# GothiProCoder/OCR-System

Measured on AMD Instinct MI355X. Metric: pages/sec end-to-end det+rec, A4@200DPI, higher is better.
Workload: dtype bf16; 1 GPU; end-to-end det+rec, batch=64 A4@200DPI pages per GPU (BASELINE configs[3]); pages_per_gpu=64, global_batch=64, lines_last_step=3279, pages_gathered_last_step=64, parallelism=pages sharded dp1, 1 all-gather/step, ranks=1, input=pages pre-decoded (uint8 RGB) and resident in HBM when the timed region starts, det_sub_batch=64

## Files before the change

### ocr-system_amd/csrc/capi.hip

```cpp
#include <cstdlib>
#include <cstring>
#include <new>

#include "../../include/lumina_ocr.h"
#include "dbpost.h"
#include "deskew.h"
#include "engine.h"
#include "marks.h"
#include "barcodes.h"
#include "qrcodes.h"
#include "datamatrix.h"
#include "aztec.h"
#include "ops.h"
#include "orient.h"
#include "resize.h"
#include "runs.h"
#include "jpeg.h"
#include "jpegdec.h"
#include "lzw.h"
#include "pngdec.h"
#include "ccitt.h"
#include "stem_conv.h"
#include "tables.h"

// ... 67 lines not shown
    return for_page_groups(h, n, fit_group(h->post_group, n, ws), ws, [&](int b0, int nb) {
        CodeGroup<T> g{};
        g.rgb = pages_dev + (size_t)b0 * height * width * 3; g.nb = nb;
        g.codes = codes_dev + (size_t)b0 * max_codes * 12; g.data = data_dev + (size_t)b0 * max_codes * row_len; g.counts = counts_dev + b0;
        g.slot_counts = slot_counts_dev ? slot_counts_dev + b0 : nullptr;
        g.mask_in = mask_in_dev ? reinterpret_cast<const unsigned long long*>(mask_in_dev) + (size_t)b0 * height * nw : nullptr;
        g.mask_out = mask_out_dev ? reinterpret_cast<unsigned long long*>(mask_out_dev) + (size_t)b0 * height * nw : nullptr;
        return hip_rc(h, what, launch(g, h->ws.get(), h->ws.cap));
    });
    API_CATCH(h)
}

extern "C" {

const char* lumina_ocr_version(void) { return "lumina-ocr-mi355x 0.1 (gfx950)"; }

int lumina_ocr_create(int device, lumina_ocr_t** out) {
    if (!out) return 1;
    *out = nullptr;
    lumina_ocr* eng = new (std::nothrow) lumina_ocr();
    if (!eng) return 1;
    eng->device = device;
    int ndev = 0;
    if (hipGetDeviceCount(&ndev) != hipSuccess || device < 0 || device >= ndev) {
        eng->err = "no HIP device " + std::to_string(device) + " (device count " + std::to_string(ndev) + ")";
        *out = eng;
        return 2;
    }
    if (hipSetDevice(device) != hipSuccess) { eng->err = "hipSetDevice failed"; *out = eng; return 2; }
    if (const char* e = getenv("LUMINA_RING_ORIENT")) eng->ring_orient = atoi(e) < 0 ? -1 : (atoi(e) != 0);
    if (getenv("LUMINA_CONV_NO_RING")) eng->conv_ring = false;
    if (getenv("LUMINA_BLOCKED")) eng->blocked_layout = atoi(getenv("LUMINA_BLOCKED")) != 0;
    *out = eng;
    return 0;
}

void lumina_ocr_destroy(lumina_ocr_t* h) {
    if (!h) return;
    (void)hipSetDevice(h->device);
    delete h;
}

const char* lumina_ocr_last_error(const lumina_ocr_t* h) { return h ? h->err.c_str() : "null handle"; }

int lumina_ocr_set_option(lumina_ocr_t* h, const char* key, int value) {
    if (!h || !key) return 1;
    if (!strcmp(key, "det_sub_batch")) h->det_sub_batch = value > 0 ? value : 1;
    else if (!strcmp(key, "rec_sub_batch")) h->rec_sub_batch = value > 0 ? value : 1;
    else if (!strcmp(key, "cls_sub_batch")) h->cls_sub_batch = value > 0 ? value : 1;
    else if (!strcmp(key, "keep_taps")) h->keep_taps = value < 0 || value > 2 ? 0 : value;
    else if (!strcmp(key, "time_convs")) h->time_convs = value != 0;
    else if (!strcmp(key, "fuse_head")) h->fuse_head = value != 0;
    else if (!strcmp(key, "fuse_mb")) h->fuse_mb = value != 0;
    else if (!strcmp(key, "fuse_pool")) h->fuse_pool = value != 0;
    else if (!strcmp(key, "fuse_stem")) h->fuse_stem = value != 0;
    else if (!strcmp(key, "fpn_multi")) h->fpn_multi = value != 0;
    else if (!strcmp(key, "fpn_compose")) h->fpn_compose = value != 0;
    else if (!strcmp(key, "fuse_short")) h->fuse_short = value != 0;
    else if (!strcmp(key, "conv_ring")) h->conv_ring = value != 0;
    else if (!strcmp(key, "blocked_layout")) h->blocked_layout = value != 0;
    else if (!strcmp(key, "conv_big_min")) h->conv_big_min = value >= 0 ? value : 1024;
    else if (!strcmp(key, "ring_orient")) h->ring_orient = value < 0 ? -1 : (value != 0);
    else if (!strcmp(key, "post_group")) h->post_group = value > 0 ? value : 1;
    else if (!strcmp(key, "tail_group")) h->tail_group = value > 0 ? value : 0;
    else if (!strcmp(key, "svtr_f16")) h->svtr_f16 = value < 0 ? -1 : (value != 0);
    else if (!strcmp(key, "png_sub_batch_mb")) h->pd_sub_batch_mb = value > 0 ? value : 1;
    else if (!strcmp(key, "conv2d_variant")) h->conv2d_variant = value < 0 || value > 2 ? 0 : value;
    else return locr_fail(h, "set_option: unknown key", key);
    return 0;
}

int lumina_ocr_load_det_weights(lumina_ocr_t* h, const void* blob, size_t nbytes) {
    if (!h || !blob) return 1;
    BIND(h);
    API_TRY return eng_load_det(h, blob, nbytes); API_CATCH(h)
}
int lumina_ocr_load_rec_weights(lumina_ocr_t* h, const void* blob, size_t nbytes) {
    if (!h || !blob) return 1;
    BIND(h);
    API_TRY return eng_load_rec(h, blob, nbytes); API_CATCH(h)
}
int lumina_ocr_num_classes(const lumina_ocr_t* h) { return h ? h->num_classes : 0; }

int lumina_ocr_normalize(lumina_ocr_t* h, const uint8_t* img_dev, int n, int height, int width, int hp, int wp, const float scale[3],
                         const float shift[3], int layout_nchw, uint16_t* out_dev, void* stream) {
    if (!h || !img_dev || !out_dev || hp < height || wp < width) return locr_fail(h, "normalize", "bad arguments");
    BIND(h);
    return hip_rc(h, "normalize", normalize_launch(img_dev, out_dev, n, height, width, hp, wp, height, width, scale, shift, layout_nchw, (hipStream_t)stream));
}

int lumina_ocr_det_forward(lumina_ocr_t* h, const uint8_t* pages_dev, int batch, int height, int width, int hp, int wp, uint16_t* prob_dev,
                           void* stream) {
    if (!h || !pages_dev || !prob_dev) return locr_fail(h, "det_forward", "null argument");
    BIND(h);
    API_TRY return eng_det_forward(h, pages_dev, batch, height, width, hp, wp, prob_dev, (hipStream_t)stream); API_CATCH(h)
}

int lumina_ocr_det_postprocess(lumina_ocr_t* h, const uint16_t* prob_dev, int batch, int hp, int wp, int valid_h, int valid_w, float thresh,
                               float box_thresh, float unclip_ratio, int min_size, int max_boxes, int32_t* boxes_dev, float* scores_dev,
                               int32_t* counts_dev, void* stream) {
    if (!h || !prob_dev || !boxes_dev || !scores_dev || !counts_dev) return locr_fail(h, "det_postprocess", "null argument");
    if (batch <= 0 || max_boxes <= 0 || valid_h > hp || valid_w > wp) return locr_fail(h, "det_postprocess", "bad dimensions");
    BIND(h);
    API_TRY
    return for_page_groups(h, batch, h->post_group, [&](int nb) { return dbpost_workspace_bytes(nb, hp, wp, max_boxes); }, [&](int b0, int nb) {
        DbPostParams p{};
// ... 750 lines not shown
```

### ocr-system_amd/csrc/conv_mfma.h

```cpp
#pragma once
#include "common.h"

enum ConvOutMode : int {
    OUT_NORMAL = 0,
    OUT_UPSAMPLE = 1,
    OUT_CONVT = 2,
    OUT_CONVT1 = 3,
    OUT_POOL = 4,
};

struct ConvParams {
    const bf16_t* x;
    const bf16_t* wpk;
    const float* bias;
    const bf16_t* res;
    bf16_t* y;
    int N, H, W, Cin;
    int Ho, Wo;
    int Cout;
    int y_cstride, y_coff;
    int res_cstride, res_h, res_w, res_shift;
    int act;
    int out_mode, up_shift, convt_c;
    int tiles_x, tiles_y, n_tiles;
    const bf16_t* fuse_w;
    float fuse_b;
    const bf16_t* gate;
    int gate_hw;
    int dbg_skip;
    int pix_limit;
    const bf16_t* zeros;
    int x_blk, y_blk, res_blk;
    int n_src;
    const bf16_t* xs[4];
    int xs_shift[4];
    int xs_nchunk[4], xs_cstride[4];
    const bf16_t* wpk2;
    const float* bias2;
    bf16_t* y2;
    int y2_cstride;
};

struct ConvKernelCfg {
    int ks, stride, bn, ck, tw, nw;
};

size_t conv_packed_weight_elems(int cout_gemm, int ks, int cin, int bn);
void pack_conv_weights(const bf16_t* ohwi, int cout_gemm, int ks, int cin, int bn, int ck, bf16_t* out, int row_major = 0);

bool conv_pick_cfg(int ks, int stride, int cin, int cout_gemm, ConvKernelCfg* cfg);
hipError_t conv_launch(const ConvKernelCfg& cfg, ConvParams p, hipStream_t stream);
const char* conv_kernel_name(const ConvKernelCfg& cfg);

bool conv_ring_supported(const ConvKernelCfg& cfg, const ConvParams& p);
bool conv_ring_transposed(const ConvParams& p, int orientation);
hipError_t conv_ring_launch(ConvParams p, int orientation, hipStream_t stream);
const char* conv_ring_kernel_name(const ConvParams& p, int orientation);

bool conv_pw_supported(const ConvKernelCfg& cfg, const ConvParams& p);
hipError_t conv_pw_launch(const ConvParams& p, hipStream_t stream);
```

### ocr-system_amd/csrc/conv_mfma.hip

```cpp
#include "conv_mfma.h"

#include <cstdlib>

namespace {

template <int KS, int S, int BN, int CK, int TW, int NW = 4, int DB = 0, int MT = 2>
struct Cfg {
    static constexpr int NTHR = NW * 64;
    static constexpr bool DMA = (DB == 3 || DB == 4);
    static constexpr bool POOL = (DB == 4);
    static constexpr bool SC = (DB == 5);
    static_assert(!SC || (KS == 3 && S == 2 && CK == 16), "fused shortcut: the 3x3 / stride-2 block-entry kernel");
    static constexpr int TH = NW * MT;
    static constexpr int PAD = (KS == 3) ? 1 : 0;
    static constexpr int HH = (TH - 1) * S + KS;
    static constexpr int HW = (TW - 1) * S + KS;
    static constexpr int HWP = HW;
    static constexpr int NPL = CK / 8;
    static constexpr int HPX = HH * HWP;
    static constexpr int PMOD = (NPL >= 8) ? 2 : 4;
    static constexpr int PLANE_A = HPX + ((PMOD - HPX % 16) + 16) % 16;
    static constexpr int TAPS = KS * KS;
    static constexpr int WROWS = TAPS * BN;
    static constexpr int PLANE_W = WROWS;
    static constexpr int NT = BN / 32;
    static constexpr int A_BYTES = DMA ? HPX * NPL * 16 : PLANE_A * NPL * 16;
    static constexpr int W_BYTES = PLANE_W * NPL * 16;
    static constexpr int W2_ROWS = SC ? 4 * BN : 0, W2_ITEMS = W2_ROWS * NPL, W2IT = (W2_ITEMS + NTHR - 1) / NTHR, W2_BYTES = W2_ITEMS * 16;
    static constexpr int A_PIX = DMA ? NPL * 16 : 16, A_SL = DMA ? 16 : PLANE_A * 16;
    static constexpr int W_ROW = DMA ? NPL * 16 : 16, W_SL = DMA ? 16 : PLANE_W * 16;
    static constexpr int STAGE_PITCH = BN * 2 + 16;
    static constexpr int STAGE_BYTES = TH * TW * STAGE_PITCH;
    static constexpr int BUF_BYTES = A_BYTES + W_BYTES + W2_BYTES;
    static constexpr int LDS_BYTES = (BUF_BYTES * (DMA ? 2 : 1)) > STAGE_BYTES ? (BUF_BYTES * (DMA ? 2 : 1)) : STAGE_BYTES;
    static_assert(!DMA || (CK == 16 && KS == 3 && S == 1), "DMA variant: 3x3 / stride 1 / 16-channel chunks");
    static constexpr int A_ITEMS = HH * HW * NPL;
    static constexpr int AIT = (A_ITEMS + NTHR - 1) / NTHR;
    static constexpr int W_ITEMS = WROWS * NPL;
    static constexpr int WIT = (W_ITEMS + NTHR - 1) / NTHR;
    static constexpr int CPP = BN / 8;
};

__device__ __forceinline__ bf16x8_t lds_frag(const unsigned char* p) { return *reinterpret_cast<const bf16x8_t*>(p); }

__device__ __forceinline__ uint32_t mul_bf16x2(uint32_t a, uint32_t b) {
    const float lo = __uint_as_float(a << 16) * __uint_as_float(b << 16);
    const float hi = __uint_as_float(a & 0xFFFF0000u) * __uint_as_float(b & 0xFFFF0000u);
    return pack_bf16x2(lo, hi);
}
__device__ __forceinline__ uint4 mul_bf16x8(uint4 a, uint4 b) {
    return make_uint4(mul_bf16x2(a.x, b.x), mul_bf16x2(a.y, b.y), mul_bf16x2(a.z, b.z), mul_bf16x2(a.w, b.w));
}

template <int KS, int S, int BN, int CK, int TW, int NW, int DB, int MT>
__global__ __launch_bounds__(NW * 64, (BN <= 64 ? 2 : 1)) void conv_mfma_kernel(const ConvParams p) {
    using C = Cfg<KS, S, BN, CK, TW, NW, DB, MT>;
    constexpr int NTHR = C::NTHR;
    extern __shared__ __attribute__((aligned(16))) unsigned char smem[];

    const int tid = threadIdx.x, lane = tid & 63, wave = tid >> 6;
    unsigned char* sA = smem;
    unsigned char* sW = sA + C::A_BYTES;
    const int r = lane & 31, h = lane >> 5;

    const int lid = xcd_remap(blockIdx.x, gridDim.x);
    const int ntile = lid % p.n_tiles;
    const int mtile = lid / p.n_tiles;
    const int tiles_per_img = p.tiles_x * p.tiles_y;
    const int n_img = mtile / tiles_per_img;
    const int trem = mtile - n_img * tiles_per_img;
    const int tile_y = trem / p.tiles_x, tile_x = trem - tile_y * p.tiles_x;

    const bf16_t* ximg = p.x + (size_t)n_img * p.H * p.W * p.Cin;
    const int nchunks = p.Cin / CK;
    const bf16_t* wbase = p.wpk + (size_t)ntile * nchunks * C::W_ITEMS * 8;

    const bool blk_dbg = CK == 16 && (p.dbg_skip & 8);
    const int pstride = blk_dbg ? 16 : p.Cin;
    const int cadv = blk_dbg ? p.H * p.W * 16 : CK;
    int a_goff[C::AIT], a_loff[C::AIT];
    int a_gate[KS == 1 ? C::AIT : 1];
    constexpr bool pool = C::POOL;
    const int oyb = pool ? tile_y * (C::TH - 2) - 1 : tile_y * C::TH, oxb = pool ? tile_x * (TW - 2) - 1 : tile_x * TW;
    const int iy0 = oyb * S - C::PAD, ix0 = oxb * S - C::PAD;
#pragma unroll
    for (int it = 0; it < C::AIT; ++it) {
        const int i = tid + NTHR * it;
        const int pi = i / C::NPL, c = i - pi * C::NPL;
        const int hy = pi / C::HW, hx = pi - hy * C::HW;
        const int iy = iy0 + hy, ix = ix0 + hx;
        const bool item = i < C::A_ITEMS;
        const bool inb = item && iy >= 0 && iy < p.H && ix >= 0 && ix < p.W && (p.pix_limit == 0 || iy * p.W + ix < p.pix_limit);
        a_goff[it] = inb ? (iy * p.W + ix) * pstride + c * 8 : -1;
        a_loff[it] = item ? (c * C::PLANE_A + hy * C::HWP + hx) * 16 : -1;
        if constexpr (KS == 1) a_gate[it] = (inb && p.gate != nullptr) ? ((iy * p.W + ix) / p.gate_hw) * p.Cin + c * 8 : -1;
    }

    uint4 a_reg[C::AIT], w_reg[C::WIT];
    uint4 g_reg[KS == 1 ? C::AIT : 1];
    uint4 w2_reg[C::SC ? C::W2IT : 1];
    unsigned char* sW2 = sW + C::W_BYTES;
    const bf16_t* wbase2 = C::SC ? p.wpk2 + (size_t)ntile * nchunks * C::W2_ITEMS * 8 : nullptr;
#define ISSUE_LOADS(chunk_)                                                                          \
    {                                                                                                \
        const bf16_t* xa = ximg + (chunk_) * cadv;                                                   \
        const bool skipa_ = (p.dbg_skip & 2) && (chunk_) > 0, skipw_ = (p.dbg_skip & 1) && (chunk_) > 0; \
        _Pragma("unroll") for (int it = 0; it < C::AIT; ++it) {                                      \
            uint4 t_ = make_uint4(0, 0, 0, 0);                                                       \
            if (a_goff[it] >= 0 && !skipa_) t_ = *reinterpret_cast<const uint4*>(xa + a_goff[it]);   \
            a_reg[it] = t_;                                                                          \
            if constexpr (KS == 1) {                                                                 \
                uint4 g_ = make_uint4(0, 0, 0, 0);                                                   \
                if (a_gate[it] >= 0) g_ = *reinterpret_cast<const uint4*>(p.gate + a_gate[it] + (chunk_) * CK); \
                g_reg[it] = g_;                                                                      \
            }                                                                                        \
        }                                                                                            \
        const uint4* wsrc = reinterpret_cast<const uint4*>(wbase + (size_t)(chunk_) * C::W_ITEMS * 8); \
        _Pragma("unroll") for (int it = 0; it < C::WIT; ++it) {                                      \
            const int i = tid + NTHR * it;                                                          \
            uint4 t_ = make_uint4(0, 0, 0, 0);                                                       \
            if ((C::W_ITEMS % NTHR == 0 || i < C::W_ITEMS) && !skipw_) t_ = wsrc[i];                 \
            w_reg[it] = t_;                                                                          \
        }                                                                                            \
        if constexpr (C::SC) {                                                                       \
// ... 293 lines not shown
                        const int cy = oyb + lr, cx = oxb + lc;
                        if (cy < 0 || cy >= p.Ho || cx < 0 || cx >= p.Wo) continue;
                        const uint4 v = *reinterpret_cast<const uint4*>(stage + (lr * TW + lc) * C::STAGE_PITCH + ch * 16);
                        const uint32_t w4[4] = {v.x, v.y, v.z, v.w};
#pragma unroll
                        for (int j = 0; j < 4; ++j) {
                            m[2 * j] = fmaxf(m[2 * j], __uint_as_float(w4[j] << 16));
                            m[2 * j + 1] = fmaxf(m[2 * j + 1], __uint_as_float(w4[j] & 0xFFFF0000u));
                        }
                    }
                const uint4 o = make_uint4(pack_bf16x2(m[0], m[1]), pack_bf16x2(m[2], m[3]), pack_bf16x2(m[4], m[5]), pack_bf16x2(m[6], m[7]));
                *reinterpret_cast<uint4*>(p.y + (((size_t)n_img * Hq + py) * Wq + px) * p.y_cstride + p.y_coff + co) = o;
            }
            return;
        }
    }
#pragma unroll
    for (int k = 0; k < (C::TH * TW * C::CPP + NTHR - 1) / NTHR; ++k) {
        const int i = tid + NTHR * k;
        const int tp = i / C::CPP, ch = i - tp * C::CPP;
        if (tp >= C::TH * TW) continue;
        const int ty = tp / TW, tx = tp - ty * TW;
        const int oy = oyb + ty, ox = oxb + tx;
        const int co = ntile * BN + ch * 8;
        if (oy >= p.Ho || ox >= p.Wo || co >= cout_r8 || (p.pix_limit != 0 && oy * p.Wo + ox >= p.pix_limit)) continue;
        const uint4 v = *reinterpret_cast<const uint4*>(stage + tp * C::STAGE_PITCH + ch * 16);
        if (p.out_mode == OUT_NORMAL) {
            bf16_t* dst = p.y + (((size_t)n_img * p.Ho + oy) * p.Wo + ox) * p.y_cstride + p.y_coff + co;
            *reinterpret_cast<uint4*>(dst) = v;
        } else if (p.out_mode == OUT_UPSAMPLE) {
            const int f = 1 << p.up_shift;
            const int HoU = p.Ho << p.up_shift, WoU = p.Wo << p.up_shift;
            for (int dy = 0; dy < f; ++dy)
                for (int dx = 0; dx < f; ++dx) {
                    bf16_t* dst = p.y + (((size_t)n_img * HoU + (oy * f + dy)) * WoU + (ox * f + dx)) * p.y_cstride + p.y_coff + co;
                    *reinterpret_cast<uint4*>(dst) = v;
                }
        } else if (p.out_mode == OUT_CONVT) {
            const int q = co / p.convt_c, cc = co - q * p.convt_c;
            const int yy = 2 * oy + (q >> 1), xx = 2 * ox + (q & 1);
            bf16_t* dst = p.y + (((size_t)n_img * (2 * p.Ho) + yy) * (2 * p.Wo) + xx) * p.y_cstride + p.y_coff + cc;
            *reinterpret_cast<uint4*>(dst) = v;
        } else {
            if (ch == 0) {
                bf16_t* dst = p.y + ((size_t)n_img * (2 * p.Ho) + 2 * oy) * (size_t)(2 * p.Wo) + 2 * ox;
                *reinterpret_cast<uint32_t*>(dst) = v.x;
                *reinterpret_cast<uint32_t*>(dst + 2 * p.Wo) = v.y;
            }
        }
    }
}

template <int KS, int S, int BN, int CK, int TW, int NW = 4, int DB = 0, int MT = 2>
hipError_t launch_t(const ConvParams& p, hipStream_t stream) {
    using C = Cfg<KS, S, BN, CK, TW, NW, DB, MT>;
    auto kern = conv_mfma_kernel<KS, S, BN, CK, TW, NW, DB, MT>;
    { hipError_t e = locr_dyn_lds(reinterpret_cast<const void*>(kern), C::LDS_BYTES); if (e != hipSuccess) return e; }
    const int grid = p.N * p.tiles_x * p.tiles_y * p.n_tiles;
    hipLaunchKernelGGL(kern, dim3(grid), dim3(C::NTHR), C::LDS_BYTES, stream, p);
    return hipGetLastError();
}

}

size_t conv_packed_weight_elems(int cout_gemm, int ks, int cin, int bn) {
    const int ntiles = (cout_gemm + bn - 1) / bn;
    return (size_t)ntiles * bn * ks * ks * cin;
}

void pack_conv_weights(const bf16_t* ohwi, int cout_gemm, int ks, int cin, int bn, int ck, bf16_t* out, int row_major) {
    const int ntiles = (cout_gemm + bn - 1) / bn, taps = ks * ks, npl = ck / 8, nchunks = cin / ck;
    const size_t wrows = (size_t)taps * bn;
    if (row_major) {
        for (int nt = 0; nt < ntiles; ++nt)
            for (int chunk = 0; chunk < nchunks; ++chunk)
                for (int tap = 0; tap < taps; ++tap)
                    for (int n = 0; n < bn; ++n) {
                        const int co = nt * bn + n;
                        bf16_t* dst = out + (((size_t)nt * nchunks + chunk) * wrows + (size_t)tap * bn + n) * ck;
                        for (int j = 0; j < ck; ++j)
                            dst[j] = co < cout_gemm ? ohwi[((size_t)co * taps + tap) * cin + chunk * ck + j] : (bf16_t)0;
                    }
        return;
    }
    for (int nt = 0; nt < ntiles; ++nt)
        for (int chunk = 0; chunk < nchunks; ++chunk)
            for (int c = 0; c < npl; ++c)
                for (int tap = 0; tap < taps; ++tap)
                    for (int n = 0; n < bn; ++n) {
                        const int co = nt * bn + n;
                        bf16_t* dst = out + ((((size_t)nt * nchunks + chunk) * npl + c) * wrows + (size_t)tap * bn + n) * 8;
                        for (int j = 0; j < 8; ++j)
                            dst[j] = co < cout_gemm ? ohwi[((size_t)co * taps + tap) * cin + chunk * ck + c * 8 + j] : (bf16_t)0;
                    }
}

bool conv_pick_cfg(int ks, int stride, int cin, int cout_gemm, ConvKernelCfg* cfg) {
    if (!((ks == 1 && stride == 1) || (ks == 2 && stride == 2) || (ks == 3 && (stride == 1 || stride == 2)))) return false;
    if (cin % 16 != 0) return false;
    cfg->ks = ks; cfg->stride = stride; cfg->tw = 32; cfg->nw = 4;
    cfg->ck = (cin % 32 == 0) ? 32 : 16;
    cfg->bn = cout_gemm <= 32 ? 32 : (cout_gemm <= 64 ? 64 : 128);
    if (cfg->bn == 128) cfg->bn = 64;
    if (ks == 3 && stride == 2 && cfg->bn == 128 && cfg->ck == 32) cfg->bn = 64;
    if (stride == 2) cfg->ck = 16;
    if (const char* e = getenv("LUMINA_CONV_CKS2")) { if (stride == 2) cfg->ck = atoi(e) == 32 && cin % 32 == 0 ? 32 : 16; }
    if (ks == 3 && stride == 1 && cin == 32 && cfg->bn == 32) cfg->ck = 16;
    if (const char* e = getenv("LUMINA_CONV_CK3")) { if (ks == 3 && stride == 1 && cin >= atoi(e)) cfg->ck = 16; }
    if (const char* e = getenv("LUMINA_CONV_NW")) {
        if ((atoi(e) == 5 || atoi(e) == 6) && ks == 3 && stride == 1 && cfg->bn == 64 && cin >= 64) { cfg->nw = atoi(e); cfg->ck = 16; }
    }
    return true;
// ... 49 lines not shown
```

### ocr-system_amd/csrc/engine.h

```cpp
#pragma once
#include <map>
#include <memory>
#include <string>
#include <type_traits>
#include <vector>

#include "common.h"
#include "conv_mfma.h"
#include "mbconv.h"
#include "svtr.h"

struct Tensor4 {
    bf16_t* p = nullptr;
    int n = 0, h = 0, w = 0, c = 0;
    bool blk = false;
    int n_src = 0; const bf16_t* xs[4] = {nullptr, nullptr, nullptr, nullptr}; int xs_shift[4] = {0, 0, 0, 0};
    int xs_c[4] = {0, 0, 0, 0}, xs_cs[4] = {0, 0, 0, 0};
    int src_c(int k) const { return xs_c[k] ? xs_c[k] : c / n_src; }
    int src_cs(int k) const { return xs_cs[k] ? xs_cs[k] : src_c(k); }
    size_t elems() const { return (size_t)n * h * w * c; }
};

struct ConvLayer {
    std::string name;
// ... 57 lines not shown
        hipError_t e = in_use ? hipEventSynchronize(in_use) : hipDeviceSynchronize();
        if (e != hipSuccess) return e;
        mem.reset(); cap = 0;
        if ((e = mem_alloc(&mem, bytes)) != hipSuccess) return e;
        cap = bytes;
        return hipSuccess;
    }
};

struct LaunchRecord { Event e0, e1; double flop, bytes; std::string layer, kernel; };

struct HostBlobTensor { int dtype; std::vector<int> dims; const uint8_t* data; size_t nbytes; };

struct lumina_ocr {
    int device = 0;
    std::string err;
    bool det_loaded = false;
    std::map<std::string, ConvLayer> det;
    bf16_t* stem_wpk = nullptr; float* stem_bias = nullptr;
    bool rec_loaded = false;
    int num_classes = 0, ctc_ntiles = 0;
    bf16_t* rstem_wpk = nullptr; float* rstem_bias = nullptr;
    std::vector<RecBlock> rblocks;
    ConvLayer rconv2, xproj[2];
    bf16_t* whh[2] = {nullptr, nullptr};
    bf16_t* ctc_wpk = nullptr; float* ctc_bias = nullptr;
    SvtrModel svtr;
    bool cls_loaded = false;
    bf16_t* cstem_wpk = nullptr; float* cstem_bias = nullptr;
    std::vector<RecBlock> cblocks;
    ConvLayer cconv2;
    float *cls_fc_w = nullptr, *cls_fc_b = nullptr;
    Growable<DeviceMem> ws;
    Arena arena;
    std::vector<DeviceMem> owned;
    bf16_t* zeros = nullptr;
    int det_sub_batch = 16, rec_sub_batch = 4096, cls_sub_batch = 4096, post_group = 64;
    int tail_group = 16;
    std::map<std::string, Tensor4> taps;
    int keep_taps = 0;
    bool fuse_head = true;
    bool fuse_pool = true;
    int conv_big_min = 1024;
    bool blocked_layout = true;
    bool conv_ring = true;
    int svtr_f16 = -1;
    int conv2d_variant = 0;
    int ring_orient = -1;
    bool fuse_short = true;
    bool fpn_compose = true;
    bool fpn_multi = true;
    bool fuse_stem = true;
    bool fuse_mb = true;
    bool time_convs = false;
    std::vector<LaunchRecord> launches;
    struct Coeffs { int ksize = 0; int* bounds = nullptr; int* kk = nullptr; std::shared_ptr<std::vector<int>> bounds_host; };
    std::map<std::pair<int, int>, Coeffs> coeff_cache;
    Growable<DeviceMem> aux;
    Growable<DeviceMem> sums;
    int jd_last_passes = 0;
    struct Staging { Growable<PinnedMem> buf; Event uploaded; };
    Staging jd_stage[2];
    int jd_stage_next = 0;
    Staging pd_stage;
    int pd_sub_batch_mb = 768;
    float* dk_trig = nullptr; short* dk_wtab = nullptr;
};

int locr_fail(lumina_ocr* eng, const char* what, const char* detail);
bool parse_blob(lumina_ocr* eng, const void* blob, size_t n, std::map<std::string, HostBlobTensor>* out);

int eng_load_det(lumina_ocr* eng, const void* blob, size_t n);
int eng_load_rec(lumina_ocr* eng, const void* blob, size_t n);
int eng_det_forward(lumina_ocr* eng, const uint8_t* pages, int B, int H, int W, int Hp, int Wp, bf16_t* prob, hipStream_t st);
int eng_rec_forward(lumina_ocr* eng, const uint8_t* crops, const int* widths, int N, int* idx, float* prob, hipStream_t st);
int eng_load_svtr(lumina_ocr* eng, const void* blob, size_t n);
int eng_load_cls(lumina_ocr* eng, const void* blob, size_t n);
int eng_cls_forward(lumina_ocr* eng, const uint8_t* crops, const int* widths, int N, float thresh, int* label, float* score, int* flip, hipStream_t st);
int eng_svtr_forward(lumina_ocr* eng, const uint8_t* crops, const int* widths, int N, int* idx, float* prob, hipStream_t st);
int eng_ws_reserve(lumina_ocr* eng, size_t bytes);
void* eng_upload(lumina_ocr* eng, const void* host, size_t bytes);
struct ConvCall {
    const Tensor4* res = nullptr; int res_shift = 0;
    int out_mode = OUT_NORMAL, up_shift = 0;
    int y_cstride = 0, y_coff = 0;
    bool flat = false;
    const bf16_t* gate = nullptr;
    const ConvLayer* short_l = nullptr; Tensor4* short_y = nullptr;
    int variant = 0;
    ConvCall& residual(const Tensor4* r, int shift = 0) { res = r; res_shift = shift; return *this; }
    ConvCall& mode(int m) { out_mode = m; return *this; }
    ConvCall& upsample(int shift) { out_mode = OUT_UPSAMPLE; up_shift = shift; return *this; }
    ConvCall& channel_slice(int cstride, int coff) { y_cstride = cstride; y_coff = coff; return *this; }
    ConvCall& flat_gemm(bool on = true) { flat = on; return *this; }
    ConvCall& gated(const bf16_t* g) { gate = g; return *this; }
    ConvCall& shortcut(const ConvLayer* l, Tensor4* y) { short_l = l; short_y = y; return *this; }
};
int eng_run_conv(lumina_ocr* eng, const ConvLayer& L, const Tensor4& x, Tensor4* y, hipStream_t st, const ConvCall& c = {});
```

### ocr-system_amd/csrc/engine.hip

```cpp
#include "engine.h"

#include <cstdlib>
#include <cstring>

#include "ops.h"
#include "stem_conv.h"

int locr_fail(lumina_ocr* eng, const char* what, const char* detail) {
    if (eng) eng->err = std::string(what) + ": " + (detail ? detail : "");
    return 1;
}

#define RUN(expr) do { if ((expr) != 0) return 1; } while (0)

#include <mutex>
#include <set>
hipError_t locr_dyn_lds(const void* kernel, int bytes) {
    static std::mutex mu;
    static std::set<std::pair<int, const void*>> done;
    int dev = 0;
    hipError_t e = hipGetDevice(&dev);
    if (e != hipSuccess) return e;
    std::lock_guard<std::mutex> lk(mu);
    if (done.count({dev, kernel})) return hipSuccess;
// ... 234 lines not shown
        if (!make_conv(eng, m, "head.convt3", 1, 1, 64, 4, 64, 4, ACT_SIGMOID, &L3, 4)) return 1;
        L3.convt = true; L3.convt_c = 1;
        const HostBlobTensor *w3, *b3;
        if (!get_wb(eng, m, "head.convt3", &w3, &b3)) return 1;
        ConvLayer& Lf = eng->det["head.convt2.fused"];
        Lf = L;
        Lf.name = "head.convt2+3";
        {
            const bf16_t* w3s = reinterpret_cast<const bf16_t*>(w3->data);
            std::vector<bf16_t> img(4 * 2 * 32 * 8, 0);
            for (int ks = 0; ks < 4; ++ks)
                for (int hh = 0; hh < 2; ++hh)
                    for (int row = 0; row < 4; ++row)
                        for (int j = 0; j < 8; ++j) img[((ks * 2 + hh) * 32 + row) * 8 + j] = w3s[row * 64 + ks * 16 + hh * 8 + j];
            Lf.fuse_w = static_cast<bf16_t*>(eng_upload(eng, img.data(), img.size() * sizeof(bf16_t)));
        }
        Lf.fuse_b = reinterpret_cast<const float*>(b3->data)[0];
        if (!Lf.fuse_w) return locr_fail(eng, "upload", "head.convt3 fused weights");
    }
    eng->det_loaded = true;
    return 0;
}

static bool conv_takes_big(const lumina_ocr* eng, const ConvLayer& L, int n, int ho, int wo, bool flat) {
    static const bool no_big = getenv("LUMINA_CONV_NO_BIG") != nullptr;
    static const long long big_min_env = getenv("LUMINA_CONV_BIG_MIN") ? atoll(getenv("LUMINA_CONV_BIG_MIN")) : -1;
    const long long nb_eff = n > eng->det_sub_batch ? n : eng->det_sub_batch;
    const long long big_blocks = nb_eff * ((ho + 15) / 16) * ((wo + 31) / 32) * ((L.cout + L.cfg.bn - 1) / L.cfg.bn);
    const long long big_min = big_min_env >= 0 ? big_min_env : eng->conv_big_min;
    return !no_big && !flat && L.wpk_big != nullptr && big_blocks >= big_min;
}

struct LaunchTimer {
    lumina_ocr* eng; hipStream_t st; Event e0, e1;
    LaunchTimer(lumina_ocr* e, hipStream_t s, bool enabled = true) : eng(e), st(s) {
        if (!enabled || !e->time_convs) return;
        hipEvent_t a = nullptr, b = nullptr;
        if (hipEventCreate(&a) == hipSuccess) e0.reset(a);
        if (hipEventCreate(&b) == hipSuccess) e1.reset(b);
        if (!e0 || !e1 || hipEventRecord(e0.get(), st) != hipSuccess) { e0.reset(); e1.reset(); }
    }
    bool on() const { return e1 != nullptr; }
    void done(std::string layer, std::string kernel, double flop, double bytes) {
        if (!on() || hipEventRecord(e1.get(), st) != hipSuccess) return;
        eng->launches.push_back(LaunchRecord{std::move(e0), std::move(e1), flop, bytes, std::move(layer), std::move(kernel)});
    }
};

static int conv_params(lumina_ocr* eng, const ConvLayer& L, const Tensor4& x, const Tensor4& y, const ConvCall& c, ConvParams* out) {
    ConvParams p{};
    p.zeros = zero_block(eng);
    if (!p.zeros) return locr_fail(eng, "conv", "zero block upload failed");
    p.gate = c.gate; p.gate_hw = x.h * x.w;
    p.x = x.p; p.wpk = L.wpk; p.bias = L.bias; p.res = c.res ? c.res->p : nullptr; p.y = y.p;
    p.Cin = L.cin; p.Cout = L.cout; p.act = L.act;
    p.out_mode = c.out_mode; p.up_shift = c.up_shift; p.convt_c = L.convt_c;
    p.fuse_w = (c.out_mode == OUT_CONVT) ? L.fuse_w : nullptr; p.fuse_b = L.fuse_b;
    if (c.flat) {
        const long long m = (long long)x.n * x.h * x.w;
        p.N = 1; p.W = 32; p.H = (int)((m + 31) / 32); p.pix_limit = (int)m;
        p.Ho = p.H; p.Wo = 32;
        p.res_h = p.H; p.res_w = 32;
    } else {
        p.N = x.n; p.H = x.h; p.W = x.w; p.pix_limit = 0;
        p.Ho = (L.ks == 3) ? (x.h - 1) / L.stride + 1 : x.h / L.stride;
        p.Wo = (L.ks == 3) ? (x.w - 1) / L.stride + 1 : x.w / L.stride;
        if (c.res) { p.res_h = c.res->h; p.res_w = c.res->w; }
    }
    p.res_shift = c.res_shift;
    p.x_blk = x.blk; p.y_blk = y.blk; p.res_blk = c.res ? c.res->blk : 0;
    p.n_src = x.n_src;
    for (int k = 0; k < 4; ++k) {
        p.xs[k] = x.xs[k]; p.xs_shift[k] = x.xs_shift[k];
        p.xs_nchunk[k] = k < x.n_src ? x.src_c(k) / 16 : 0; p.xs_cstride[k] = k < x.n_src ? x.src_cs(k) : 0;
    }
    p.res_cstride = c.res ? c.res->c : 0;
    p.y_cstride = c.y_cstride ? c.y_cstride : y.c;
    p.y_coff = c.y_coff;
    if (const ConvLayer* s = c.short_l) {
        const Tensor4* sy = c.short_y;
        if (sy == nullptr || s->cin != L.cin || s->cout != L.cout || s->cfg.bn != L.cfg.bn || s->cfg.ck != L.cfg.ck || s->ks != 2 || s->stride != 2 ||
            sy->c != L.cout || sy->h != y.h || sy->w != y.w)
            return locr_fail(eng, "fused shortcut: layer mismatch", L.name.c_str());
        p.wpk2 = s->wpk; p.bias2 = s->bias; p.y2 = sy->p; p.y2_cstride = sy->c;
    }
    if (x.c != L.cin) return locr_fail(eng, "conv input channels mismatch", L.name.c_str());
    *out = p;
    return 0;
}

enum ConvKernel { CONV_TILE_8X32, CONV_TILE_16X32, CONV_POINTWISE, CONV_RING };
struct ConvChoice { ConvKernel kernel; ConvKernelCfg cfg; const bf16_t* wpk; };

static int conv_choose(lumina_ocr* eng, const ConvLayer& L, const ConvParams& p, const ConvCall& c, ConvChoice* out) {
    if (p.out_mode == OUT_POOL && (L.wpk_big == nullptr || L.cfg_big.nw != 6)) return locr_fail(eng, "fused max pool needs the LDS-DMA conv kernel", L.name.c_str());
    const bool forced = c.variant != 0 && L.wpk_big != nullptr;
    const bool big = forced || p.out_mode == OUT_POOL || p.n_src > 1 || conv_takes_big(eng, L, p.N, p.Ho, p.Wo, c.flat);
    if (forced && c.variant == 2 && !conv_ring_supported(L.cfg_big, p)) return locr_fail(eng, "conv2d_variant 2: the ring kernel does not take this layer", L.name.c_str());
    *out = big ? ConvChoice{CONV_TILE_16X32, L.cfg_big, L.wpk_big} : ConvChoice{CONV_TILE_8X32, L.cfg, L.wpk};
    static const bool no_pw = getenv("LUMINA_CONV_NO_PW") != nullptr;
    const bool ring_on = c.variant == 0 ? eng->conv_ring : c.variant == 2;
    if (!no_pw && !big && conv_pw_supported(out->cfg, p)) out->kernel = CONV_POINTWISE;
    else if (ring_on && big && conv_ring_supported(out->cfg, p)) out->kernel = CONV_RING;
    if (p.n_src > 1 && out->kernel != CONV_RING) return locr_fail(eng, "a multi-source input reached a kernel other than the ring kernel", L.name.c_str());
    if (out->kernel != CONV_RING && (p.x_blk || p.y_blk || p.res_blk)) return locr_fail(eng, "a channel-blocked tensor reached a kernel that cannot address it", L.name.c_str());
    return 0;
// ... 663 lines not shown
```

Measured before the change: 1627 pages/sec.

## Add direct-load 1x1 conv path with register-streamed activations and whole-K weight slab

Adds a direct path for 1x1 stride-1 convolutions. Activations are streamed from global memory into registers through buffer loads with a multi-stage prefetch, and the full K-range weight slab (plus an optional SE gate) is staged in LDS once. This removes the per-chunk LDS staging and barriers of the generic kernel for Cin values that fit poorly. The path is gated by a heuristic on Cin and LDS size. Launch-bounds occupancy for small-BN 1x1 kernels is also raised, which may increase register pressure or spilling.

```diff
diff --git a/ocr-system_amd/csrc/capi.hip b/ocr-system_amd/csrc/capi.hip
--- a/ocr-system_amd/csrc/capi.hip
+++ b/ocr-system_amd/csrc/capi.hip
@@ -143,6 +143,7 @@
     else if (!strcmp(key, "time_convs")) h->time_convs = value != 0;
     else if (!strcmp(key, "fuse_head")) h->fuse_head = value != 0;
     else if (!strcmp(key, "fuse_mb")) h->fuse_mb = value != 0;
+    else if (!strcmp(key, "conv1x1_direct")) h->conv1x1_direct = value != 0;
     else if (!strcmp(key, "fuse_pool")) h->fuse_pool = value != 0;
     else if (!strcmp(key, "fuse_stem")) h->fuse_stem = value != 0;
     else if (!strcmp(key, "fpn_multi")) h->fpn_multi = value != 0;
diff --git a/ocr-system_amd/csrc/conv_mfma.h b/ocr-system_amd/csrc/conv_mfma.h
--- a/ocr-system_amd/csrc/conv_mfma.h
+++ b/ocr-system_amd/csrc/conv_mfma.h
@@ -27,6 +27,7 @@
     float fuse_b;
     const bf16_t* gate;
     int gate_hw;
+    int direct1x1;
     int dbg_skip;
     int pix_limit;
     const bf16_t* zeros;
diff --git a/ocr-system_amd/csrc/conv_mfma.hip b/ocr-system_amd/csrc/conv_mfma.hip
--- a/ocr-system_amd/csrc/conv_mfma.hip
+++ b/ocr-system_amd/csrc/conv_mfma.hip
@@ -52,8 +52,208 @@
     return make_uint4(mul_bf16x2(a.x, b.x), mul_bf16x2(a.y, b.y), mul_bf16x2(a.z, b.z), mul_bf16x2(a.w, b.w));
 }
 
+constexpr int D1X1 = 4;
+constexpr int DIRECT1X1_MAX_LDS = 65536;
+
+__device__ __forceinline__ bool conv1x1_pixel(const ConvParams& p, int oyb, int oxb, int row, int r, int* pix, int* oy, int* ox) {
+    const int y = oyb + row, x = oxb + r;
+    const bool valid = y < p.H && x < p.W && (p.pix_limit == 0 || y * p.W + x < p.pix_limit);
+    *oy = valid ? y : oyb; *ox = valid ? x : oxb;
+    *pix = *oy * p.W + *ox;
+    return valid;
+}
+
+template <int BN, int MT, bool GATED>
+__device__ __forceinline__ void conv1x1_direct_body(const ConvParams& p, unsigned char* sW, int ntile, int n_img, int oyb, int oxb) {
+    constexpr int NT = BN / 32, D = D1X1;
+    static_assert(D % 2 == 0, "the A-fragment double buffer alternates with the k-step");
+    const int tid = threadIdx.x, lane = tid & 63, wave = tid >> 6, r = lane & 31, h = lane >> 5;
+    const int nks = p.Cin >> 4;
+
+    const int pix0 = oyb * p.W + oxb, img_px = p.pix_limit ? p.pix_limit : p.H * p.W;
+    const long long xbytes = (long long)(img_px - pix0) * p.Cin * 2;
+    const auto xrs = __builtin_amdgcn_make_buffer_rsrc(const_cast<bf16_t*>(p.x + ((size_t)n_img * p.H * p.W + pix0) * p.Cin), 0,
+                                                       (int)(xbytes < 0x7FFFFFFFLL ? xbytes : 0x7FFFFFFFLL), 0x00020000);
+    unsigned char* sG = sW + p.Cin * BN * 2;
+    const int crop0 = GATED ? pix0 / p.gate_hw : 0;
+    int kbyte = 0;
+    uint32_t xo[MT], go[GATED ? MT : 1];
+#pragma unroll
+    for (int mt = 0; mt < MT; ++mt) {
+        int pix, oy, ox;
+        conv1x1_pixel(p, oyb, oxb, wave * MT + mt, r, &pix, &oy, &ox);
+        xo[mt] = (uint32_t)((pix - pix0) * p.Cin + 8 * h) * 2u;
+        if constexpr (GATED) go[mt] = (uint32_t)((pix / p.gate_hw - crop0) * p.Cin + 8 * h) * 2u;
+    }
+
+    uint4 xb[D][MT];
+#define LOAD_K(d_, koff_)                                                                            \
+    {                                                                                                \
+        _Pragma("unroll") for (int mt = 0; mt < MT; ++mt) {                                          \
+            xb[d_][mt] = __builtin_bit_cast(uint4, __builtin_amdgcn_raw_buffer_load_b128(xrs, xo[mt], kbyte + (koff_) * 32, 0)); \
+        }                                                                                            \
+    }
+#pragma unroll
+    for (int d = 0; d < D; ++d)
+        if (d < nks) LOAD_K(d, d)
+
+    if constexpr (GATED) {
+        int last_y = oyb + 7 < p.H ? oyb + 7 : p.H - 1, last_x = oxb + 31 < p.W ? oxb + 31 : p.W - 1;
+        int last = last_y * p.W + last_x;
+        if (last > img_px - 1) last = img_px - 1;
+        const int gitems = (last / p.gate_hw - crop0 + 1) * (p.Cin >> 3);
+        const uint4* gsrc = reinterpret_cast<const uint4*>(p.gate + (size_t)crop0 * p.Cin);
+        for (int i = tid; i < gitems; i += 256) *reinterpret_cast<uint4*>(sG + (size_t)i * 16) = gsrc[i];
+    }
+    const int witems = p.Cin * (BN / 8);
+    const uint4* wsrc = reinterpret_cast<const uint4*>(p.wpk + (size_t)ntile * p.Cin * BN);
+    int i0 = 0;
+    do {
+        uint4 t[4];
+#pragma unroll
+        for (int u = 0; u < 4; ++u) { const int i = i0 + u * 256 + tid; t[u] = wsrc[i < witems ? i : witems - 1]; }
+#pragma unroll
+        for (int u = 0; u < 4; ++u) {
+            const int i = i0 + u * 256 + tid;
+            *reinterpret_cast<uint4*>(sW + (size_t)(i < witems ? i : witems - 1) * 16) = t[u];
+        }
+    } while ((i0 += 4 * 256) < witems);
+    __syncthreads();
+
+    f32x16_t acc[MT][NT];
+#pragma unroll
+    for (int mt = 0; mt < MT; ++mt)
+#pragma unroll
+        for (int nt = 0; nt < NT; ++nt)
+#pragma unroll
+            for (int j = 0; j < 16; ++j) acc[mt][nt][j] = 0.f;
+
+    const unsigned char* wfrag = sW + (h * BN + r) * 16;
+    bf16x8_t afr[2][NT];
+    uint4 gfr[GATED ? 2 : 1][GATED ? MT : 1];
+#define LOAD_A(set_, ks_)                                                                            \
+    {                                                                                                \
+        const int ka_ = (ks_) < nks ? (ks_) : nks - 1;                                               \
+        _Pragma("unroll") for (int nt = 0; nt < NT; ++nt) afr[set_][nt] = lds_frag(wfrag + (2 * ka_ * BN + nt * 32) * 16); \
+        if constexpr (GATED) { _Pragma("unroll") for (int mt = 0; mt < MT; ++mt) gfr[set_][mt] = *reinterpret_cast<const uint4*>(sG + go[mt] + ka_ * 32); } \
+    }
+#define STEP_K(d_, ks_)                                                                              \
+    {                                                                                                \
+        LOAD_A(((d_) + 1) & 1, (ks_) + 1)                                                            \
+        _Pragma("unroll") for (int mt = 0; mt < MT; ++mt) {                                          \
+            uint4 b_ = xb[d_][mt];                                                                   \
+            if constexpr (GATED) b_ = mul_bf16x8(b_, gfr[(d_) & 1][mt]);                             \
+            const bf16x8_t bf_ = __builtin_bit_cast(bf16x8_t, b_);                                   \
+            _Pragma("unroll") for (int nt = 0; nt < NT; ++nt)                                        \
+                acc[mt][nt] = __builtin_amdgcn_mfma_f32_32x32x16_bf16(afr[(d_) & 1][nt], bf_, acc[mt][nt], 0, 0, 0); \
+        }                                                                                            \
+    }
+    LOAD_A(0, 0)
+    int ks0 = 0;
+    for (; ks0 + 2 * D <= nks; ks0 += D) {
+#pragma unroll
+        for (int d = 0; d < D; ++d) {
+            STEP_K(d, ks0 + d)
+            if (d == D - 1) {
+#pragma unroll
+                for (int e = 0; e < D; ++e) LOAD_K(e, D + e)
+            }
+            __builtin_amdgcn_sched_barrier(0);
+        }
+        kbyte += D * 32;
+    }
+    for (; ks0 < nks; ks0 += D) {
+#pragma unroll
+        for (int d = 0; d < D; ++d)
+            if (ks0 + d < nks) {
+                STEP_K(d, ks0 + d)
+                if (ks0 + D + d < nks) LOAD_K(d, D + d)
+            }
+        kbyte += D * 32;
+    }
+#undef STEP_K
+#undef LOAD_A
+#undef LOAD_K
+
+    int lane2 = threadIdx.x;
+    asm volatile("" : "+v"(lane2));
+    const int r2 = lane2 & 31, h2 = (lane2 >> 5) & 1, wave2 = lane2 >> 6;
+    const int cout_r8 = (p.Cout + 7) & ~7;
+    const float* bptr = p.bias + ntile * BN;
+    float4 bias_r[NT][4];
+#pragma unroll
+    for (int nt = 0; nt < NT; ++nt)
+#pragma unroll
+        for (int g = 0; g < 4; ++g) bias_r[nt][g] = *reinterpret_cast<const float4*>(bptr + nt * 32 + 8 * g + 4 * h2);
+    uint2 res_r[MT][NT][4];
+    bool pvalid[MT];
+    int opix[MT];
+    const bool has_res = p.res != nullptr;
+#pragma unroll
+    for (int mt = 0; mt < MT; ++mt) {
+        int oy, ox;
+        pvalid[mt] = conv1x1_pixel(p, oyb, oxb, wave2 * MT + mt, r2, &opix[mt], &oy, &ox);
+        if (has_res) {
+            const bf16_t* rrow = p.res + (((size_t)n_img * p.res_h + (oy >> p.res_shift)) * p.res_w + (ox >> p.res_shift)) * p.res_cstride + ntile * BN;
+#pragma unroll
+            for (int nt = 0; nt < NT; ++nt)
+#pragma unroll
+                for (int g = 0; g < 4; ++g) {
+                    const int cn = nt * 32 + 8 * g + 4 * h2;
+                    uint2 rv = make_uint2(0, 0);
+                    if (ntile * BN + cn < cout_r8) rv = *reinterpret_cast<const uint2*>(rrow + cn);
+                    res_r[mt][nt][g] = rv;
+                }
+        }
+    }
+
+#pragma unroll
+    for (int mt = 0; mt < MT; ++mt)
+#pragma unroll
+        for (int nt = 0; nt < NT; ++nt)
+#pragma unroll
+            for (int g = 0; g < 4; ++g) {
+                const float4 b4 = bias_r[nt][g];
+                acc[mt][nt][4 * g + 0] += b4.x; acc[mt][nt][4 * g + 1] += b4.y;
+                acc[mt][nt][4 * g + 2] += b4.z; acc[mt][nt][4 * g + 3] += b4.w;
+                if (has_res) {
+                    const uint2 rv = res_r[mt][nt][g];
+                    acc[mt][nt][4 * g + 0] += __uint_as_float(rv.x << 16); acc[mt][nt][4 * g + 1] += __uint_as_float(rv.x & 0xFFFF0000u);
+                    acc[mt][nt][4 * g + 2] += __uint_as_float(rv.y << 16); acc[mt][nt][4 * g + 3] += __uint_as_float(rv.y & 0xFFFF0000u);
+                }
+            }
+#define FOR_ALL_ACC(expr)                                                          \
+    _Pragma("unroll") for (int mt = 0; mt < MT; ++mt)                               \
+        _Pragma("unroll") for (int nt = 0; nt < NT; ++nt)                          \
+            _Pragma("unroll") for (int j = 0; j < 16; ++j) { const float v = acc[mt][nt][j]; acc[mt][nt][j] = (expr); }
+    if (p.act == ACT_RELU) { FOR_ALL_ACC(fmaxf(v, 0.f)) }
+    else if (p.act == ACT_HSWISH) { FOR_ALL_ACC(v * fminf(fmaxf(v + 3.f, 0.f), 6.f) * (1.f / 6.f)) }
+    else if (p.act == ACT_SIGMOID) { FOR_ALL_ACC(fast_sigmoidf(v)) }
+    else if (p.act == ACT_HSIGMOID) { FOR_ALL_ACC(fminf(fmaxf(0.2f * v + 0.5f, 0.f), 1.f)) }
+    else if (p.act == ACT_GELU) { FOR_ALL_ACC(gelu_erf(v)) }
+#undef FOR_ALL_ACC
+#pragma unroll
+    for (int mt = 0; mt < MT; ++mt) {
+        bf16_t* yrow = p.y + ((size_t)n_img * p.Ho * p.Wo + opix[mt]) * p.y_cstride + p.y_coff;
+#pragma unroll
+        for (int nt = 0; nt < NT; ++nt)
+#pragma unroll
+            for (int gp2 = 0; gp2 < 2; ++gp2) {
+                const int g0 = 2 * gp2, g1 = 2 * gp2 + 1;
+                const uint32_t q0x = pack_bf16x2(acc[mt][nt][4 * g0 + 0], acc[mt][nt][4 * g0 + 1]), q0y = pack_bf16x2(acc[mt][nt][4 * g0 + 2], acc[mt][nt][4 * g0 + 3]);
+                const uint32_t q1x = pack_bf16x2(acc[mt][nt][4 * g1 + 0], acc[mt][nt][4 * g1 + 1]), q1y = pack_bf16x2(acc[mt][nt][4 * g1 + 2], acc[mt][nt][4 * g1 + 3]);
+                const auto sx = __builtin_amdgcn_permlane32_swap(q0x, q1x, false, false);
+                const auto sy = __builtin_amdgcn_permlane32_swap(q0y, q1y, false, false);
+                const uint4 v = make_uint4(sx[0], sy[0], sx[1], sy[1]);
+                const int co = ntile * BN + nt * 32 + 16 * gp2 + 8 * h2;
+                if (!pvalid[mt] || co >= cout_r8) continue;
+                *reinterpret_cast<uint4*>(yrow + co) = v;
+            }
+    }
+}
+
 template <int KS, int S, int BN, int CK, int TW, int NW, int DB, int MT>
-__global__ __launch_bounds__(NW * 64, (BN <= 64 ? 2 : 1)) void conv_mfma_kernel(const ConvParams p) {
+__global__ __launch_bounds__(NW * 64, (KS == 1 && DB == 0 && BN <= 64) ? (BN <= 32 ? 4 : 3) : (BN <= 64 ? 2 : 1)) void conv_mfma_kernel(const ConvParams p) {
     using C = Cfg<KS, S, BN, CK, TW, NW, DB, MT>;
     constexpr int NTHR = C::NTHR;
     extern __shared__ __attribute__((aligned(16))) unsigned char smem[];
@@ -70,6 +270,14 @@
     const int n_img = mtile / tiles_per_img;
     const int trem = mtile - n_img * tiles_per_img;
     const int tile_y = trem / p.tiles_x, tile_x = trem - tile_y * p.tiles_x;
+
+    if constexpr (KS == 1 && !C::DMA) {
+        if (p.direct1x1) {
+            if (p.gate != nullptr) conv1x1_direct_body<BN, MT, true>(p, smem, ntile, n_img, tile_y * C::TH, tile_x * TW);
+            else conv1x1_direct_body<BN, MT, false>(p, smem, ntile, n_img, tile_y * C::TH, tile_x * TW);
+            return;
+        }
+    }
 
     const bf16_t* ximg = p.x + (size_t)n_img * p.H * p.W * p.Cin;
     const int nchunks = p.Cin / CK;
@@ -469,12 +677,18 @@
 }
 
 template <int KS, int S, int BN, int CK, int TW, int NW = 4, int DB = 0, int MT = 2>
-hipError_t launch_t(const ConvParams& p, hipStream_t stream) {
+hipError_t launch_t(ConvParams p, hipStream_t stream) {
     using C = Cfg<KS, S, BN, CK, TW, NW, DB, MT>;
     auto kern = conv_mfma_kernel<KS, S, BN, CK, TW, NW, DB, MT>;
-    { hipError_t e = locr_dyn_lds(reinterpret_cast<const void*>(kern), C::LDS_BYTES); if (e != hipSuccess) return e; }
+    constexpr bool can_direct = KS == 1 && S == 1 && !C::DMA;
+    constexpr int max_lds = can_direct && C::LDS_BYTES < DIRECT1X1_MAX_LDS ? DIRECT1X1_MAX_LDS : C::LDS_BYTES;
+    { hipError_t e = locr_dyn_lds(reinterpret_cast<const void*>(kern), max_lds); if (e != hipSuccess) return e; }
+    const int slab = p.Cin * BN * 2 + (p.gate ? ((7 * p.W + 31) / (p.gate_hw > 0 ? p.gate_hw : 1) + 2) * p.Cin * 2 : 0);
+    const bool pays = (p.Cin % 64 != 0 && p.Cin > 16 && !(p.gate != nullptr && p.Cin >= 256)) || p.Cin >= 512;
+    p.direct1x1 = can_direct && p.direct1x1 && pays && p.out_mode == OUT_NORMAL && slab <= DIRECT1X1_MAX_LDS;
+    const int lds = p.direct1x1 ? slab : C::LDS_BYTES;
     const int grid = p.N * p.tiles_x * p.tiles_y * p.n_tiles;
-    hipLaunchKernelGGL(kern, dim3(grid), dim3(C::NTHR), C::LDS_BYTES, stream, p);
+    hipLaunchKernelGGL(kern, dim3(grid), dim3(C::NTHR), lds, stream, p);
     return hipGetLastError();
 }
 
diff --git a/ocr-system_amd/csrc/engine.h b/ocr-system_amd/csrc/engine.h
--- a/ocr-system_amd/csrc/engine.h
+++ b/ocr-system_amd/csrc/engine.h
@@ -133,6 +133,7 @@
     bool fpn_multi = true;
     bool fuse_stem = true;
     bool fuse_mb = true;
+    bool conv1x1_direct = true;
     bool time_convs = false;
     std::vector<LaunchRecord> launches;
     struct Coeffs { int ksize = 0; int* bounds = nullptr; int* kk = nullptr; std::shared_ptr<std::vector<int>> bounds_host; };
diff --git a/ocr-system_amd/csrc/engine.hip b/ocr-system_amd/csrc/engine.hip
--- a/ocr-system_amd/csrc/engine.hip
+++ b/ocr-system_amd/csrc/engine.hip
@@ -310,6 +310,7 @@
     p.zeros = zero_block(eng);
     if (!p.zeros) return locr_fail(eng, "conv", "zero block upload failed");
     p.gate = c.gate; p.gate_hw = x.h * x.w;
+    p.direct1x1 = eng->conv1x1_direct;
     p.x = x.p; p.wpk = L.wpk; p.bias = L.bias; p.res = c.res ? c.res->p : nullptr; p.y = y.p;
     p.Cin = L.cin; p.Cout = L.cout; p.act = L.act;
     p.out_mode = c.out_mode; p.up_shift = c.up_shift; p.convt_c = L.convt_c;
```

Result: no change. 1631 pages/sec, median of 6 (+0.2%).
